# VGLoic/kzg-poly-commit-exploration

Hardware: AMD Instinct MI355X
Metric: g1_msm_commitments_per_sec_degree_2^20 (higher is better)
Workload: dtype i32 digits (Fp: 13 signed radix-2^30 digits, Montgomery 2^390; Fr: 8 x u32, Montgomery 2^256)

## Files before the change

### kzg_poly_commit_exploration_amd/csrc/api.hip

```cpp
#include <hip/hip_runtime.h>
#include <sys/random.h>

#include <algorithm>
#include <atomic>
#include <cerrno>
#include <chrono>
#include <condition_variable>
#include <cstdio>
#include <cstdlib>
#include <cstring>
#include <deque>
#include <functional>
#include <mutex>
#include <new>
#include <string>
#include <thread>
#include <vector>

#include "../../include/kzg_mi355x.h"
#include "engine.h"
#include "host_field.hpp"
#include "host_fr.hpp"
#include "fr30_host.hpp"
#include "host_pairing.hpp"
#include "host_sha256.hpp"
#include "wire30.hip.h"

using namespace kzg;
namespace hf = kzg_host;

namespace {

constexpr size_t kMaxCoefficients = 0xFFFFFFFFull;

#ifndef KZG_NUM_SLOTS
#define KZG_NUM_SLOTS 5
#endif
constexpr int kNumSlots = KZG_NUM_SLOTS;
struct ReducePlan {
    uint32_t lo_bits = 0, hi_bits = 0;
    uint32_t row_lo = 0, row_hi = 0;
    uint32_t col_lo = 0, col_hi = 0;
    uint32_t off_r2row = 0, off_c2row = 0, off_r2col = 0, off_c2col = 0, total = 0;
};

enum SlotKind { SLOT_IDLE = 0, SLOT_COMMIT = 1, SLOT_OPEN = 2, SLOT_TRIVIAL = 3, SLOT_COMMIT_BATCH = 4, SLOT_OPEN_BATCH = 5, SLOT_RESERVED = 6,
                SLOT_OPEN_POINTS = 7 ,
                SLOT_OPEN_COMBINED = 8 ,
                SLOT_OPEN_SETS = 9  };

int hip_fail(kzg_ctx* ctx, const char* what, hipError_t e);

struct DevBuf {
    void* p = nullptr;
    size_t cap = 0;
    DevBuf() = default;
    DevBuf(const DevBuf&) = delete;
    DevBuf& operator=(const DevBuf&) = delete;
    ~DevBuf() { reset(); }
    void reset() {
        if (p) hipFree(p);
        p = nullptr;
        cap = 0;
    }
    template <class T = uint32_t> T* dev() const { return (T*)p; }
    int reserve(kzg_ctx* ctx, size_t bytes, hipStream_t drain = nullptr) { return bytes <= cap ? KZG_OK : grow(ctx, bytes, drain); }
    int grow(kzg_ctx* ctx, size_t bytes, hipStream_t drain) {
        if (drain)
            if (hipError_t e = hipStreamSynchronize(drain)) return hip_fail(ctx, "hipStreamSynchronize", e);
        reset();
        if (hipError_t e = hipMalloc(&p, bytes)) {
            p = nullptr;
            return hip_fail(ctx, "hipMalloc", e);
        }
// ... 74 lines not shown
    DevBuf recoded;
    DevBuf part_a, part_b;
    DevBuf pair_scratch;
    DevBuf heavy_ws;
    DevBuf arena;
    PinnedBuf fin{PinnedBuf::Mapped};
    DevBuf stage;
    DevBuf q;
    DevBuf chunk, block;
    PinnedBuf small{PinnedBuf::Mapped};
    PinnedBuf bsmall{PinnedBuf::Mapped};
    std::vector<uint32_t> open_ys;
    PinnedBuf roots{PinnedBuf::Staged};
    PinnedBuf pvals{PinnedBuf::Mapped};
    DevBuf pblock;
    std::vector<uint32_t> pts_ys;
    size_t pts_nq = 0;
    PinnedBuf ctab{PinnedBuf::Staged};
    PinnedBuf cvals{PinnedBuf::Mapped};
    DevBuf cpart, cin;
    size_t cmb_t = 0;
    float combine_ms = 0;
    PinnedBuf stab{PinnedBuf::Staged}, ssel{PinnedBuf::Staged};
    PinnedBuf svals{PinnedBuf::Mapped};
    DevBuf sg;
    std::vector<uint32_t> sets_vmap;
    PinnedBuf ltab{PinnedBuf::Staged};
    PinnedBuf btab{PinnedBuf::Staged};
    DevBuf lag_part;
    DevBuf gp_in, gp_z, gp_part;
    PinnedBuf gp_flags{PinnedBuf::Mapped};
    DevBuf cpoly, cagg;
    DevBuf ml_in, ml_pyr;
    SlotKind kind = SLOT_IDLE;
    size_t job_n = 0;
    uint32_t job_batch = 1;
    uint32_t open_y[8] = {};
    bool timing = false;
    bool has_quotient = false;
    bool tail_checked = false;
    kzg_kernel_times times = {};
};

}

struct kzg_ctx {
    kzg::MultiState* multi = nullptr;
    int device = 0;
    std::mutex mu;
    std::condition_variable slot_cv;
    int sync_owned = 0;
    bool raw_partials = false;
    bool host_trace = false;
    std::atomic<uint64_t> trace_ns[5] = {};
    std::atomic<uint64_t> trace_calls{0};
    std::string last_error;
    size_t n = 0;
    MsmConfig cfg = {};
    DevBuf table;
    bool nttb_ready = false;
    DevBuf ntt_tw;
    DevBuf lag_table;
    size_t lag_n = 0;
    uint64_t srs_gen = 0;
    ReducePlan plan;
    size_t arena_records = 0, final_records = 0;
    uint32_t max_batch = 1;
    Slot slots[kNumSlots];
    hipStream_t front_stream = nullptr, heavy_stream = nullptr, tail_stream = nullptr;
    hipStream_t upload_stream = nullptr;
    uint32_t accum_lds_bytes = 41u * 1024u;
    uint32_t small_lds_bytes = 48u * 1024u;
    bool small_msm_off = false;
    size_t pq_ws_budget = (size_t)1 << 30;
    bool slots_ready = false;
    bool timing = false;
    std::mutex fk20_mu;
    DevBuf glv;
    uint32_t glv_log = 0;
    DevBuf fk20_B, fk20_tab;
    uint32_t fk20_log_L = 0, fk20_log_l = 0;
    Workspace<11> fk20_ws;
    std::mutex recover_mu;
    DevBuf rec_g;
    Workspace<11> rec_ws;
    Workspace<17> vc_ws;
    Workspace<8> blob_ws;
    std::mutex lookup_mu;
    Workspace<6> lu_ws;
    std::mutex quotient_mu;
    Workspace<13> pq_ws;
    DevBuf prove_buf[5];
    uint32_t pq_zinv_key = ~0u;
    std::vector<kzg_circuit*> circuits;
};

struct kzg_circuit {
    kzg_ctx* owner = nullptr;
    uint32_t lg_n = 0, lg_ext = 0;
    size_t n = 0, t = 0;
    size_t c_tab = 0;
    size_t g_custom = 0, d_max = 0;
    uint8_t exps[kCgMaxTerms * kPqMaxColumns] = {};
    uint8_t exps_next[kCgMaxTerms * kPqMaxColumns] = {};
    size_t rho = 0;
    uint8_t next_wires[kPqMaxColumns] = {};
    uint64_t shifts[4 * kPqMaxColumns] = {};
    DevBuf values;
// ... 188 lines not shown

int build_tables(kzg_ctx* ctx, hipStream_t st, void* d_xyzz_tmp, void* d_prefix) {
    const size_t n = ctx->n;
    for (uint32_t j = 1; j < ctx->cfg.W; j++) {
        char* prev = (char*)ctx->table.p + (size_t)(j - 1) * n * kAffineBytes;
        char* next = (char*)ctx->table.p + (size_t)j * n * kAffineBytes;
        launch_table_window(st, prev, (uint32_t)n, ctx->cfg.level_bits, d_xyzz_tmp, d_prefix, next);
    }
    HIP_TRY(ctx, hipGetLastError());
    HIP_TRY(ctx, hipStreamSynchronize(st));
    return KZG_OK;
}

int drain_all(kzg_ctx* ctx) {
    for (hipStream_t st : {ctx->upload_stream, ctx->front_stream, ctx->heavy_stream, ctx->tail_stream})
        if (st) HIP_TRY(ctx, hipStreamSynchronize(st));
    return KZG_OK;
}

static int srs_release(kzg_ctx* ctx) {
    ctx->slots_ready = false;
    int rc = drain_all(ctx);
    if (rc) return rc;
    for (auto& s : ctx->slots) s.kind = SLOT_IDLE;
    ctx->table.reset();
    ctx->fk20_B.reset();
    ctx->fk20_tab.reset();
    ctx->lag_table.reset();
    ctx->lag_n = 0;
    ctx->srs_gen++;
    ctx->n = 0;
    return KZG_OK;
}

int srs_prepare(kzg_ctx* ctx, size_t n) {
    if (n == 0 || n > 0x7fffffffu / 32) return KZG_ERR_INVALID_ARG;
    int rc = srs_release(ctx);
    if (rc) return rc;
    size_t free_b = 0, total_b = 0;
    HIP_TRY(ctx, hipMemGetInfo(&free_b, &total_b));
    size_t budget = (size_t)((double)free_b * 0.6);
    if (const char* v = std::getenv("KZG_TABLE_GB")) budget = (size_t)(std::strtod(v, nullptr) * 1073741824.0);
    MsmConfig cfg = choose_msm_config(n, budget);
    if ((size_t)cfg.W * n >= 0x80000000ull) return KZG_ERR_INVALID_ARG;
    ctx->cfg = cfg;
    return ctx->table.reserve(ctx, (size_t)cfg.W * n * kAffineBytes);
}

struct MsmBasis {
    const void* table;
    uint32_t stride;
};
int enqueue_msm(kzg_ctx* ctx, Slot& s, const uint32_t* d_scalars, int is_mont, size_t n, int ev_base,
                uint32_t batch = 1, uint64_t stride = 0, const MsmBasis* basis = nullptr) {
    const MsmConfig cfg = ctx->cfg;
    const void* table = basis ? basis->table : ctx->table.p;
    const uint32_t table_stride = basis ? basis->stride : (uint32_t)ctx->n;
    const uint32_t nbt = cfg.nb * batch;
    hipStream_t st = s.stream;
    s.end = st;
    if (s.timing) HIP_TRY(ctx, hipEventRecord(s.ev[ev_base], st));
    const bool header_zeroed = launch_bucket_sort(st, d_scalars, is_mont, (uint32_t)n, batch, stride, table_stride, cfg, s.cnt.dev(),
                       s.block_sums.dev(), s.pairs.dev<uint64_t>(), s.recoded.dev(), s.offs.dev(), s.sorted.dev(), (uint32_t*)s.heavy_ws.p);
    if (s.timing) {
        HIP_TRY(ctx, hipEventRecord(s.ev[ev_base + 1], st));
        HIP_TRY(ctx, hipEventRecord(s.ev[ev_base + 2], st));
    }
    bool alone = true;
    for (const auto& other : ctx->slots) alone = alone && (&other == &s || other.kind == SLOT_IDLE);
    const uint64_t max_refs = (uint64_t)n * cfg.max_digits * batch;
    const uint32_t lanes = accumulate_lanes(max_refs, alone);
    const ReducePlan& P = ctx->plan;
    const uint32_t R = 1u << P.hi_bits, C = 1u << P.lo_bits, B = batch;
    char* row = (char*)s.arena.p;
    char* col = row + (size_t)R * B * kXyzzBytes;
    char* fin = (char*)s.fin.d;
    const uint32_t rl = 1u << P.row_lo, rh = 1u << P.row_hi, cl = 1u << P.col_lo, ch = 1u << P.col_hi;
    const TreeSumDesc stage1[2] = {
        {s.buckets.p, row, B * R, C, C, 1, B * R, 0},
        {s.buckets.p, col, B * C, R, 1, C, C, (uint64_t)cfg.nb}};
    const TreeSumDesc stage2[4] = {
        {row, fin + (size_t)P.off_r2row * B * kXyzzBytes, B * rh, rl, rl, 1, rh, R},
        {row, fin + (size_t)P.off_c2row * B * kXyzzBytes, B * rl, rh, 1, rl, rl, R},
        {col, fin + (size_t)P.off_r2col * B * kXyzzBytes, B * ch, cl, cl, 1, ch, C},
        {col, fin + (size_t)P.off_c2col * B * kXyzzBytes, B * cl, ch, 1, cl, cl, C}};
    if (!header_zeroed) HIP_TRY(ctx, hipMemsetAsync(s.heavy_ws.p, 0, kHeavyHeaderBytes, st));
    if (max_refs <= kTinyRefs && !ctx->small_msm_off) {
        if (s.timing) HIP_TRY(ctx, hipEventRecord(s.ev[ev_base + 3], st));
        launch_small_msm(st, table, s.sorted.dev(), s.offs.dev(), nbt, lanes, max_refs, s.buckets.p, s.part_a.p, s.part_b.p,
                         s.heavy_ws.p, s.small.dev() + 26, stage1, stage2, ctx->small_lds_bytes);
        if (s.timing) HIP_TRY(ctx, hipEventRecord(s.ev[ev_base + 4], st));
    } else {
        const bool hand_over = !alone;
        hipStream_t hs = hand_over ? ctx->heavy_stream : st;
        if (hand_over) {
            HIP_TRY(ctx, hipEventRecord(s.sorted_ev, st));
            HIP_TRY(ctx, hipStreamWaitEvent(hs, s.sorted_ev, 0));
        }
        if (s.timing) HIP_TRY(ctx, hipEventRecord(s.ev[ev_base + 3], hs));
        launch_bucket_accumulate(hs, table, s.sorted.dev(), s.offs.dev(), nbt, lanes, s.buckets.p, s.part_a.p, s.part_b.p,
                                 ctx->accum_lds_bytes, s.pair_scratch.p, max_refs,
                                 (char*)s.heavy_ws.p + kAccumClockOffset);
        if (s.timing) HIP_TRY(ctx, hipEventRecord(s.ev[ev_base + 4], hs));
        if (hand_over) {
            HIP_TRY(ctx, hipEventRecord(s.accum_ev, hs));
            st = s.end = ctx->tail_stream;
            HIP_TRY(ctx, hipStreamWaitEvent(st, s.accum_ev, 0));
        }
        launch_bucket_finalize(st, s.offs.dev(), nbt, lanes, s.part_a.p, s.part_b.p, s.buckets.p, s.heavy_ws.p, s.small.dev() + 26,
                               finalize_group_size(nbt));
        launch_tree_sums_two_stage(st, stage1, 2, stage2, 4, (uint32_t*)s.heavy_ws.p + 64, alone);
    }
    if (s.timing) HIP_TRY(ctx, hipEventRecord(s.ev[ev_base + 5], st));
    HIP_TRY(ctx, hipGetLastError());
    return KZG_OK;
}

hf::PX host_wsum(const uint64_t* recs, uint32_t len) {
    hf::PX run = hf::px_inf(), acc = hf::px_inf();
    for (uint32_t v = len; v-- > 1;) {
        run = hf::px_add(run, hf::px_from_record(recs + (size_t)v * kXyzzWords64));
        acc = hf::px_add(acc, run);
    }
    return acc;
}
hf::PX host_shift(hf::PX p, uint32_t k) {
    for (uint32_t i = 0; i < k; i++) p = hf::px_double(p);
    return p;
}
hf::P1 finish_msm(const kzg_ctx* ctx, const Slot& s, uint32_t p = 0, uint32_t batch = 1) {
    const ReducePlan& P = ctx->plan;
    const uint64_t* f = s.fin.host<uint64_t>();
    auto at = [&](uint32_t off, uint32_t len) { return f + ((size_t)off * batch + (size_t)p * len) * kXyzzWords64; };
    const uint32_t rh = 1u << P.row_hi, rl = 1u << P.row_lo, ch = 1u << P.col_hi, cl = 1u << P.col_lo;
    hf::PX w_row = hf::px_add(host_shift(host_wsum(at(P.off_r2row, rh), rh), P.row_lo), host_wsum(at(P.off_c2row, rl), rl));
    hf::PX w_col = hf::px_add(host_shift(host_wsum(at(P.off_r2col, ch), ch), P.col_lo), host_wsum(at(P.off_c2col, cl), cl));
    hf::PX total = hf::px_add(host_shift(w_row, P.lo_bits), w_col);
    if (ctx->cfg.recode == kRecodeNaf) total = hf::px_double(total);
    const uint64_t* r2 = at(P.off_r2row, rh);
    for (uint32_t k = 0; k < rh; k++) total = hf::px_add(total, hf::px_from_record(r2 + (size_t)k * kXyzzWords64));
    return ctx->raw_partials ? hf::px_to_jacobian(total) : hf::px_normalize(total);
}

void write_p1(uint64_t out[18], const hf::P1& p) { std::memcpy(out, &p, sizeof p); }

void fill_device_times(Slot& s) {
    s.times.references = s.small.host()[26];
    const uint64_t not_start = (uint64_t)s.small.host()[28] | ((uint64_t)s.small.host()[29] << 32);
    const uint64_t end = (uint64_t)s.small.host()[30] | ((uint64_t)s.small.host()[31] << 32);
    if (not_start != 0 && end > ~not_start) s.times.accumulate_ms = (float)((double)(end - ~not_start) * 1e-5);
}
void fill_accumulate_times(Slot& s) {
    float ms = 0;
    (void)hipEventElapsedTime(&ms, s.ev[3], s.ev[4]);
    s.times.accumulate_events_ms = ms;
    if (s.times.accumulate_ms == 0) s.times.accumulate_ms = ms;
}

void slot_idle(kzg_ctx* ctx, Slot& s) {
    s.kind = SLOT_IDLE;
    ctx->slot_cv.notify_all();
}
int reserve_slot(kzg_ctx* ctx, std::unique_lock<std::mutex>& lk, bool block) {
    for (;;) {
        for (int i = 0; i < kNumSlots; i++)
            if (ctx->slots[i].kind == SLOT_IDLE) {
                ctx->slots[i].kind = SLOT_RESERVED;
                ctx->sync_owned++;
                return i;
            }
        if (!block || ctx->sync_owned == 0) return -1;
        ctx->slot_cv.wait(lk);
    }
}
void release_owned(kzg_ctx* ctx, int slot) {
    if (ctx->slots[slot].kind == SLOT_RESERVED) ctx->slots[slot].kind = SLOT_IDLE;
    ctx->sync_owned--;
    ctx->slot_cv.notify_all();
}
struct SlotLease {
    kzg_ctx* ctx;
    int slot;
    ~SlotLease() { if (slot >= 0) release_owned(ctx, slot); }
};
void quiesce(kzg_ctx* ctx, std::unique_lock<std::mutex>& lk) {
    while (ctx->sync_owned > 0) ctx->slot_cv.wait(lk);
}

bool host_tail_nonzero(const uint64_t* coeffs, size_t from, size_t n) {
    for (size_t i = from; i < n; i++)
        if (coeffs[4 * i] | coeffs[4 * i + 1] | coeffs[4 * i + 2] | coeffs[4 * i + 3]) return true;
    return false;
}
// ... 70 lines not shown
        case KZG_ERR_CONSTANT_POLY: return "Unable to divide a constant polynomial";
        case KZG_ERR_REMAINDER:
            return "[divide_by_root] Fail to divide the polynomial by a root, constant terms do not add up";
        case KZG_ERR_INVALID_ARG: return "invalid argument";
        case KZG_ERR_NO_DEVICE: return "no HIP device available (this library has no CPU path)";
        case KZG_ERR_HIP: return "HIP runtime error";
        case KZG_ERR_NO_SRS: return "no SRS loaded";
        case KZG_ERR_BUSY: return "slot busy";
        default: return "unknown status";
    }
}

const char* kzg_last_error(const kzg_ctx* ctx) {
    if (!ctx) return "";
    if (ctx->multi && ctx->last_error.empty()) return multi_last_error(ctx->multi);
    return ctx->last_error.c_str();
}

int kzg_ctx_create_multi_ex(const int* devices, int ndev, unsigned flags, kzg_ctx** out) {
    if (!out) return KZG_ERR_INVALID_ARG;
    *out = nullptr;
    if (!devices || ndev <= 0 || (flags & ~(unsigned)KZG_MULTI_REPLICATE_SRS)) return KZG_ERR_INVALID_ARG;
    kzg::MultiState* m = nullptr;
    std::string err;
    int rc = multi_create(devices, ndev, (flags & KZG_MULTI_REPLICATE_SRS) ? kMultiReplicate : kMultiRange, &m, err);
    if (rc != KZG_OK) return rc;
    kzg_ctx* ctx = new kzg_ctx();
    ctx->multi = m;
    ctx->device = devices[0];
    *out = ctx;
    return KZG_OK;
}
int kzg_ctx_create_multi(const int* devices, int ndev, kzg_ctx** out) { return kzg_ctx_create_multi_ex(devices, ndev, 0u, out); }
int kzg_abi_version(void) { return KZG_ABI_VERSION; }
int kzg_num_devices(const kzg_ctx* ctx) { return !ctx ? 0 : (ctx->multi ? multi_num_devices(ctx->multi) : 1); }
uint64_t kzg_rccl_exchanges(const kzg_ctx* ctx) { return (ctx && ctx->multi) ? multi_rccl_exchanges(ctx->multi) : 0; }

int kzg_ctx_create(int device, kzg_ctx** out) {
    if (!out) return KZG_ERR_INVALID_ARG;
    *out = nullptr;
    int count = 0;
    if (hipGetDeviceCount(&count) != hipSuccess || count <= 0) return KZG_ERR_NO_DEVICE;
    if (device < 0 || device >= count) return KZG_ERR_NO_DEVICE;
    if (hipSetDevice(device) != hipSuccess) return KZG_ERR_NO_DEVICE;
    kzg_ctx* ctx = new kzg_ctx();
    ctx->device = device;
    if (const char* v = std::getenv("KZG_ACCUM_LDS_KB")) ctx->accum_lds_bytes = (uint32_t)std::atoi(v) * 1024u;
    if (const char* v = std::getenv("KZG_SMALL_MSM")) ctx->small_msm_off = std::atoi(v) == 0;
    if (const char* v = std::getenv("KZG_PQ_WS_KB")) {
        const long kb = std::atol(v);
        ctx->pq_ws_budget = kb < 0 ? 0 : (kb > (1l << 20) ? (size_t)1 << 30 : (size_t)kb * 1024);
    }
    if (const char* v = std::getenv("KZG_HOST_TRACE")) ctx->host_trace = std::atoi(v) != 0;
    if (hipFuncSetAttribute(small_msm_kernel(), hipFuncAttributeMaxDynamicSharedMemorySize, (int)small_msm_lds_bytes()) == hipSuccess)
        ctx->small_lds_bytes = small_msm_lds_bytes();
    else
        (void)hipGetLastError();
    if (!poly_prepare_device() || !points_prepare_device() || !sets_prepare_device()) {
        delete ctx;
        return KZG_ERR_HIP;
    }
    *out = ctx;
    return KZG_OK;
}

void kzg_ctx_destroy(kzg_ctx* ctx) {
    if (!ctx) return;
    if (ctx->multi) {
        multi_destroy(ctx->multi);
        delete ctx;
        return;
    }
    hipSetDevice(ctx->device);
    if (ctx->host_trace && ctx->trace_calls.load()) {
        const double k = 1e-3 / (double)ctx->trace_calls.load();
        std::fprintf(stderr, "[kzg host trace] %llu kzg_commit calls, us per call: wait-for-slot %.1f upload %.1f submit %.1f device %.1f collect %.1f\n",
                     (unsigned long long)ctx->trace_calls.load(), k * ctx->trace_ns[0].load(), k * ctx->trace_ns[1].load(),
                     k * ctx->trace_ns[2].load(), k * ctx->trace_ns[3].load(), k * ctx->trace_ns[4].load());
    }
    for (hipStream_t st : {ctx->upload_stream, ctx->front_stream, ctx->heavy_stream, ctx->tail_stream})
        if (st) hipStreamSynchronize(st);
    for (hipStream_t st : {ctx->upload_stream, ctx->front_stream, ctx->heavy_stream, ctx->tail_stream})
        if (st) hipStreamDestroy(st);
    for (kzg_circuit* c : ctx->circuits) delete c;
    delete ctx;
}

size_t kzg_srs_len(const kzg_ctx* ctx) { return !ctx ? 0 : (ctx->multi ? multi_srs_len(ctx->multi) : ctx->n); }
int kzg_num_slots(const kzg_ctx*) { return kNumSlots; }

int kzg_msm_config(const kzg_ctx* ctx, int* digit_bits, int* table_levels, size_t* num_buckets, int* recoding) {
    if (ctx && ctx->multi)
        return kzg_msm_config(multi_kid(ctx->multi, 0), digit_bits, table_levels, num_buckets, recoding);
    if (!ctx || !ctx->n) return KZG_ERR_NO_SRS;
    if (digit_bits) *digit_bits = (int)ctx->cfg.c;
    if (table_levels) *table_levels = (int)ctx->cfg.W;
    if (num_buckets) *num_buckets = ctx->cfg.nb;
    if (recoding) *recoding = (int)ctx->cfg.recode;
    return KZG_OK;
}

int kzg_srs_load_g1(kzg_ctx* ctx, const void* first_g1, size_t stride, size_t n) {
    if (!ctx || !first_g1 || stride < 144) return KZG_ERR_INVALID_ARG;
    if (ctx->multi) {
        std::lock_guard<std::mutex> lkm(ctx->mu);
        ctx->last_error.clear();
        return n ? multi_srs_load(ctx->multi, first_g1, stride, n) : KZG_ERR_INVALID_ARG;
    }
    std::unique_lock<std::mutex> lk(ctx->mu);
    quiesce(ctx, lk);
    HIP_TRY(ctx, hipSetDevice(ctx->device));
    int rc = srs_prepare(ctx, n);
    if (rc) return rc;
    std::vector<uint64_t> packed(n * 18);
    for (size_t i = 0; i < n; i++) std::memcpy(&packed[i * 18], (const char*)first_g1 + i * stride, 144);
    DevBuf d_jac, d_prefix, d_xyzz;
    HIP_TRY(ctx, hipMalloc(&d_jac.p, n * 144));
    HIP_TRY(ctx, hipMalloc(&d_prefix.p, n * 64));
    HIP_TRY(ctx, hipMalloc(&d_xyzz.p, n * kXyzzBytes));
    TmpStream st;
    HIP_TRY(ctx, hipStreamCreateWithFlags(&st.s, hipStreamNonBlocking));
    HIP_TRY(ctx, hipMemcpyAsync(d_jac.p, packed.data(), n * 144, hipMemcpyHostToDevice, st.s));
    ctx->n = n;
    launch_jacobian_to_affine(st.s, d_jac.p, (uint32_t)n, ctx->table.p, d_prefix.p);
    rc = build_tables(ctx, st.s, d_xyzz.p, d_prefix.p);
    if (rc) {
        ctx->n = 0;
        return rc;
    }
    return setup_slots(ctx);
}
// ... 196 lines not shown
    if (ok) {
        ok = std::fseek(f, 0, SEEK_END) == 0;
        const long end = ok ? std::ftell(f) : -1;
        ok = ok && end >= 0 && (uint64_t)end == 128ull + 96ull * h.n && std::fseek(f, 128, SEEK_SET) == 0;
    }
    std::vector<uint64_t> xy;
    if (ok) {
        try {
            xy.resize((size_t)h.n * 12);
        } catch (const std::bad_alloc&) {
            std::fclose(f);
            return fail("out of host memory for the SRS file");
        }
        ok = std::fread(xy.data(), 96, h.n, f) == h.n;
    }
    std::fclose(f);
    if (ok) {
        uint8_t a[48], b[48];
        affine96_compress(xy.data(), a);
        affine96_compress(&xy[12 * ((size_t)h.n - 1)], b);
        ok = std::memcmp(a, h.first, 48) == 0 && std::memcmp(b, h.last, 48) == 0;
    }
    if (!ok) return fail("not a KZGSRS1 file, truncated, or its fingerprint does not match its content");
    size_t bad = 0;
    if (!affine96_all_on_curve(xy.data(), (size_t)h.n, &bad)) return fail("SRS file: point " + std::to_string(bad) + " is not on the curve");
    return kzg_srs_load_affine(ctx, xy.data(), (size_t)h.n);
}

int kzg_srs_read_g1(kzg_ctx* ctx, size_t index, size_t count, uint64_t* out_p1) {
    if (!ctx || !out_p1) return KZG_ERR_INVALID_ARG;
    std::lock_guard<std::mutex> lk(ctx->mu);
    if (ctx->multi) return multi_srs_len(ctx->multi) ? multi_srs_read(ctx->multi, index, count, out_p1) : KZG_ERR_NO_SRS;
    if (!ctx->n) return KZG_ERR_NO_SRS;
    if (index > ctx->n || count > ctx->n - index) return KZG_ERR_INVALID_ARG;
    if (!count) return KZG_OK;
    HIP_TRY(ctx, hipSetDevice(ctx->device));
    DevBuf d_p1;
    HIP_TRY(ctx, hipMalloc(&d_p1.p, count * 144));
    hipStream_t st = ctx->slots[0].stream;
    launch_affine_to_p1(st, (const char*)ctx->table.p + index * kAffineBytes, (uint32_t)count, d_p1.p);
    HIP_TRY(ctx, hipMemcpyAsync(out_p1, d_p1.p, count * 144, hipMemcpyDeviceToHost, st));
    HIP_TRY(ctx, hipStreamSynchronize(st));
    return KZG_OK;
}


static bool lagrange_basis(const kzg_ctx* ctx, size_t n, MsmBasis* out) {
    if (!ctx->lag_table.p || ctx->lag_n != n) return false;
    *out = MsmBasis{ctx->lag_table.p, (uint32_t)ctx->lag_n};
    return true;
}

static int submit_commit_locked(kzg_ctx* ctx, int slot, const uint32_t* d_scalars, int is_mont, size_t n,
                                bool tail_already_checked, bool owned = false, const MsmBasis* basis = nullptr) {
    if (!ctx->n || !ctx->slots_ready) return KZG_ERR_NO_SRS;
    if (basis && (basis->stride != n || n > ctx->n)) return KZG_ERR_INVALID_ARG;
    if (slot < 0 || slot >= kNumSlots) return KZG_ERR_INVALID_ARG;
    Slot& s = ctx->slots[slot];
    if (s.kind != (owned ? SLOT_RESERVED : SLOT_IDLE)) return KZG_ERR_BUSY;
    HIP_TRY(ctx, hipSetDevice(ctx->device));
    s.timing = ctx->timing;
    s.end = s.stream;
    s.has_quotient = false;
    s.job_n = n;
    s.job_batch = 1;
    s.tail_checked = tail_already_checked;
    std::memset(&s.times, 0, sizeof s.times);
    size_t n_msm = n < ctx->n ? n : ctx->n;
    std::memset(s.small.host(), 0, 64 * 4);
    if (n > ctx->n && !tail_already_checked) {
        uint64_t cnt = n - ctx->n;
        hipLaunchKernelGGL(k_tail_nonzero, dim3((unsigned)((cnt + 255) / 256)), dim3(256), 0, s.stream, d_scalars,
                           (uint64_t)ctx->n, (uint64_t)n, s.small.dev() + 24);
    }
    if (n_msm == 0) {
        s.kind = SLOT_TRIVIAL;
        return KZG_OK;
    }
    int rc = enqueue_msm(ctx, s, d_scalars, is_mont, n_msm, 0, 1, 0, basis);
    if (rc) return rc;
    HIP_TRY(ctx, hipEventRecord(s.done, s.end));
    s.kind = SLOT_COMMIT;
    return KZG_OK;
}

int kzg_commit_submit(kzg_ctx* ctx, int slot, const void* d_coeffs, size_t n) {
    KZG_SINGLE_DEVICE_ONLY(ctx);
    if (!ctx || (!d_coeffs && n)) return KZG_ERR_INVALID_ARG;
    if (n > kMaxCoefficients) return KZG_ERR_INVALID_ARG;
    std::lock_guard<std::mutex> lk(ctx->mu);
    return submit_commit_locked(ctx, slot, (const uint32_t*)d_coeffs, 1, n, false);
}

static int submit_open_locked(kzg_ctx* ctx, int slot, const uint32_t* d_coeffs, size_t n, const uint64_t z[4],
                              const uint64_t y[4], bool owned = false) {
    if (!ctx->n || !ctx->slots_ready) return KZG_ERR_NO_SRS;
    if (slot < 0 || slot >= kNumSlots) return KZG_ERR_INVALID_ARG;
    Slot& s = ctx->slots[slot];
    if (s.kind != (owned ? SLOT_RESERVED : SLOT_IDLE)) return KZG_ERR_BUSY;
    HIP_TRY(ctx, hipSetDevice(ctx->device));
    int rc = ensure_poly(ctx, s, n);
    if (rc) return rc;
    s.timing = ctx->timing;
    s.end = s.stream;
    s.job_n = n;
    s.job_batch = 1;
    s.has_quotient = true;
    s.tail_checked = false;
    std::memcpy(s.open_y, y, 32);
    std::memset(&s.times, 0, sizeof s.times);
    if (n == 0) {
        std::memset(s.small.host(), 0, 64 * 4);
        s.kind = SLOT_TRIVIAL;
        return KZG_OK;
    }
    uint32_t zw[8];
    std::memcpy(zw, z, 32);
    if (s.timing) HIP_TRY(ctx, hipEventRecord(s.ev[6], s.stream));
    if (!launch_quotient_single(s.stream, d_coeffs, (uint32_t)n, zw, n > 1 ? s.q.dev() : nullptr, s.small.dev())) {
        std::memset(s.small.host(), 0, 64 * 4);
        PolyScratch sc{s.chunk.dev(), s.block.dev(), s.small.dev(), s.small.dev() + 8};
        launch_quotient(s.stream, d_coeffs, (uint32_t)n, zw, n > 1 ? s.q.dev() : nullptr, sc);
    }
    if (s.timing) HIP_TRY(ctx, hipEventRecord(s.ev[7], s.stream));
    size_t nq = n - 1;
    if (nq > ctx->n) {
        uint64_t from = ctx->n + 1, cnt = n - from;
        hipLaunchKernelGGL(k_tail_nonzero, dim3((unsigned)((cnt + 255) / 256)), dim3(256), 0, s.stream, d_coeffs, from,
                           (uint64_t)n, s.small.dev() + 24);
        nq = ctx->n;
    }
    if (nq > 0) {
// ... 13 lines not shown
    return submit_open_locked(ctx, slot, (const uint32_t*)d_coeffs, n, z, y);
}

static int submit_points_locked(kzg_ctx* ctx, int slot, const uint32_t* d_coeffs, size_t n, const uint64_t* zs,
                                const uint64_t* ys, size_t k, bool owned = false) {
    if (!ctx->n || !ctx->slots_ready) return KZG_ERR_NO_SRS;
    if (slot < 0 || slot >= kNumSlots) return KZG_ERR_INVALID_ARG;
    Slot& s = ctx->slots[slot];
    if (s.kind != (owned ? SLOT_RESERVED : SLOT_IDLE)) return KZG_ERR_BUSY;
    uint64_t ws[4 * KZG_MAX_OPEN_POINTS];
    int rc = points_weights(ctx, zs, k, ws);
    if (rc) return rc;
    HIP_TRY(ctx, hipSetDevice(ctx->device));
    rc = ensure_poly(ctx, s, n);
    if (rc == KZG_OK) rc = ensure_points(ctx, s, n, k);
    if (rc) return rc;
    s.timing = ctx->timing;
    s.end = s.stream;
    s.job_n = n;
    s.job_batch = 1;
    s.has_quotient = true;
    s.tail_checked = false;
    s.pts_ys.assign((const uint32_t*)ys, (const uint32_t*)ys + 8 * k);
    std::memset(&s.times, 0, sizeof s.times);
    size_t nq = n > k ? n - k : 0;
    if (s.timing) HIP_TRY(ctx, hipEventRecord(s.ev[6], s.stream));
    rc = enqueue_points_scan(ctx, s, d_coeffs, n, zs, ws, k, nq, nq > 0);
    if (rc) return rc;
    if (s.timing) HIP_TRY(ctx, hipEventRecord(s.ev[7], s.stream));
    if (nq > ctx->n) {
        const uint64_t from = ctx->n + k, cnt = n - from;
        hipLaunchKernelGGL(k_tail_nonzero, dim3((unsigned)((cnt + 255) / 256)), dim3(256), 0, s.stream, d_coeffs, from,
                           (uint64_t)n, s.small.dev() + 24);
        nq = ctx->n;
    }
    if (nq > 0) {
        rc = enqueue_msm(ctx, s, s.q.dev(), 1, nq, 0);
        if (rc) return rc;
    }
    s.pts_nq = nq;
    HIP_TRY(ctx, hipEventRecord(s.done, s.end));
    s.kind = SLOT_OPEN_POINTS;
    return KZG_OK;
}

int kzg_open_points_submit(kzg_ctx* ctx, int slot, const void* d_coeffs, size_t n, const uint64_t* zs, const uint64_t* ys,
                           size_t k) {
    KZG_SINGLE_DEVICE_ONLY(ctx);
    if (!ctx || !zs || !ys || (!d_coeffs && n) || n > kMaxCoefficients) return KZG_ERR_INVALID_ARG;
    std::lock_guard<std::mutex> lk(ctx->mu);
    return submit_points_locked(ctx, slot, (const uint32_t*)d_coeffs, n, zs, ys, k);
}

static int wait_locked(kzg_ctx* ctx, int slot, uint64_t out_p1[18]) {
    if (slot < 0 || slot >= kNumSlots) return KZG_ERR_INVALID_ARG;
    Slot& s = ctx->slots[slot];
    if (s.kind == SLOT_IDLE) return KZG_ERR_INVALID_ARG;
    if (s.kind == SLOT_COMMIT_BATCH || s.kind == SLOT_OPEN_BATCH) {
        ctx->last_error = "kzg_wait on a slot that holds a batched job (use kzg_wait_batch / kzg_wait_open_batch)";
        return KZG_ERR_INVALID_ARG;
    }
    if (s.kind == SLOT_OPEN_COMBINED) {
        ctx->last_error = "kzg_wait on a slot that holds a combined opening (use kzg_wait_combined)";
        return KZG_ERR_INVALID_ARG;
    }
    if (s.kind == SLOT_OPEN_SETS) {
        ctx->last_error = "kzg_wait on a slot that holds an opening at several point sets (use kzg_wait_sets)";
        return KZG_ERR_INVALID_ARG;
    }
    if (s.kind == SLOT_RESERVED) return KZG_ERR_BUSY;
    HIP_TRY(ctx, hipSetDevice(ctx->device));
    SlotKind kind = s.kind;
    slot_idle(ctx, s);
    HIP_TRY(ctx, hipEventSynchronize(s.done));
    const bool ran_msm = kind != SLOT_TRIVIAL && !(kind == SLOT_OPEN_POINTS && s.pts_nq == 0);
    if (ran_msm) fill_device_times(s);
    if (s.timing && ran_msm) {
        float ms = 0;
        hipEventElapsedTime(&ms, s.ev[0], s.ev[1]); s.times.digits_ms = ms;
        hipEventElapsedTime(&ms, s.ev[2], s.ev[3]); s.times.scatter_ms = ms;
        fill_accumulate_times(s);
        hipEventElapsedTime(&ms, s.ev[4], s.ev[5]); s.times.reduce_ms = ms;
        if (s.has_quotient) {
            hipEventElapsedTime(&ms, s.ev[6], s.ev[7]); s.times.quotient_ms = ms;
            hipEventElapsedTime(&ms, s.ev[6], s.ev[5]); s.times.total_ms = ms;
        } else {
            hipEventElapsedTime(&ms, s.ev[0], s.ev[5]); s.times.total_ms = ms;
        }
    }
    const uint32_t* hs = s.small.host();
    hf::P1 inf = hf::p1_inf();
    if (kind == SLOT_OPEN_POINTS) {
        const size_t k = s.pts_ys.size() / 8;
        const uint32_t* vals = points_values(s, k);
        for (size_t i = 0; i < k; i++)
            if (std::memcmp(vals + 8 * i, s.pts_ys.data() + 8 * i, 32) != 0) return KZG_ERR_REMAINDER;
        if (hs[24]) return KZG_ERR_DEGREE_TOO_HIGH;
        write_p1(out_p1, s.pts_nq ? finish_msm(ctx, s) : inf);
        return KZG_OK;
    }
    if (s.has_quotient) {
        const size_t n = s.job_n;
        if (n == 0) {
            bool y_zero = true;
            for (int i = 0; i < 8; i++) y_zero &= s.open_y[i] == 0;
            if (!y_zero) return KZG_ERR_CONSTANT_POLY;
            write_p1(out_p1, inf);
            return KZG_OK;
        }
        bool higher_nonzero = hs[0] & 1u;
        if (!higher_nonzero) {
            if (std::memcmp(hs + 16, s.open_y, 32) != 0) return KZG_ERR_CONSTANT_POLY;
            write_p1(out_p1, inf);
            return KZG_OK;
        }
        if (std::memcmp(hs + 8, s.open_y, 32) != 0) return KZG_ERR_REMAINDER;
        if (hs[24]) return KZG_ERR_DEGREE_TOO_HIGH;
    } else {
        if (hs[24]) return KZG_ERR_DEGREE_TOO_HIGH;
    }
    if (kind == SLOT_TRIVIAL) {
        write_p1(out_p1, inf);
        return KZG_OK;
    }
    write_p1(out_p1, finish_msm(ctx, s));
    return KZG_OK;
}

int kzg_set_max_batch(kzg_ctx* ctx, size_t max_batch) {
    if (!ctx || max_batch == 0) return KZG_ERR_INVALID_ARG;
    if (ctx->multi) return multi_set_max_batch(ctx->multi, max_batch);
    std::unique_lock<std::mutex> lk(ctx->mu);
    quiesce(ctx, lk);
    HIP_TRY(ctx, hipSetDevice(ctx->device));
    int rc = drain_all(ctx);
    if (rc) return rc;
    for (auto& s : ctx->slots)
        if (s.kind != SLOT_IDLE) return KZG_ERR_BUSY;
    const uint32_t previous = ctx->max_batch;
    ctx->max_batch = (uint32_t)(max_batch > 1024 ? 1024 : max_batch);
    if (!ctx->n) return KZG_OK;
    rc = setup_slots(ctx, true);
    if (rc != KZG_OK) {
        const std::string why = ctx->last_error;
        ctx->max_batch = previous;
        (void)hipGetLastError();
        (void)setup_slots(ctx);
        ctx->last_error = why;
    }
    return rc;
}

size_t kzg_max_batch(const kzg_ctx* ctx) {
    if (ctx && ctx->multi) return kzg_max_batch(multi_kid(ctx->multi, 0));
    return ctx ? ctx->max_batch : 0;
}

static int commit_batch_submit_locked(kzg_ctx* ctx, int slot, const void* d_coeffs, size_t n, size_t batch,
                                      size_t stride_coeffs, bool owned = false, bool lagrange = false) {
    if (!ctx->n || !ctx->slots_ready) return KZG_ERR_NO_SRS;
    MsmBasis basis{};
    if (lagrange && !lagrange_basis(ctx, n, &basis)) return KZG_ERR_NO_SRS;
    if (slot < 0 || slot >= kNumSlots || batch > ctx->max_batch) return KZG_ERR_INVALID_ARG;
    if (n > ctx->n) return KZG_ERR_DEGREE_TOO_HIGH;
    Slot& s = ctx->slots[slot];
    if (s.kind != (owned ? SLOT_RESERVED : SLOT_IDLE)) return KZG_ERR_BUSY;
    HIP_TRY(ctx, hipSetDevice(ctx->device));
    s.timing = ctx->timing;
    s.end = s.stream;
    s.has_quotient = false;
    s.job_n = n;
    s.job_batch = (uint32_t)batch;
    s.tail_checked = true;
// ... 122 lines not shown
    const hf::P1 inf = hf::p1_inf();
    for (uint32_t p = 0; p < B; p++) {
        const uint32_t* hs = s.bsmall.host() + p * 32;
        const uint32_t* y = s.open_ys.data() + 8 * p;
        uint64_t* out = out_p1s + out_stride * (size_t)p;
        int& status = statuses[status_stride * (size_t)p];
        if (!(hs[0] & 1u)) {
            if (std::memcmp(hs + 16, y, 32) != 0) status = KZG_ERR_CONSTANT_POLY;
            else { status = KZG_OK; write_p1(out, inf); }
            continue;
        }
        if (std::memcmp(hs + 8, y, 32) != 0) { status = KZG_ERR_REMAINDER; continue; }
        status = KZG_OK;
        write_p1(out, finish_msm(ctx, s, p, B));
    }
    s.open_ys.clear();
    return KZG_OK;
}

int kzg_wait_open_batch(kzg_ctx* ctx, int slot, uint64_t* out_p1s, int* statuses, size_t batch) {
    KZG_SINGLE_DEVICE_ONLY(ctx);
    if (!ctx || !out_p1s || !statuses) return KZG_ERR_INVALID_ARG;
    std::lock_guard<std::mutex> lk(ctx->mu);
    return wait_open_batch_locked(ctx, slot, out_p1s, statuses, batch);
}

int kzg_wait(kzg_ctx* ctx, int slot, uint64_t out_p1[18]) {
    KZG_SINGLE_DEVICE_ONLY(ctx);
    if (!ctx || !out_p1) return KZG_ERR_INVALID_ARG;
    std::lock_guard<std::mutex> lk(ctx->mu);
    return wait_locked(ctx, slot, out_p1);
}


static void await_unlocked(std::unique_lock<std::mutex>& lk, Slot& s) {
    if (s.kind == SLOT_TRIVIAL || s.kind == SLOT_RESERVED || s.kind == SLOT_IDLE) return;
    lk.unlock();
    (void)hipEventSynchronize(s.done);
    lk.lock();
}

struct HostTrace {
    kzg_ctx* ctx;
    std::chrono::steady_clock::time_point t;
    explicit HostTrace(kzg_ctx* c) : ctx(c) { if (c->host_trace) t = std::chrono::steady_clock::now(); }
    void mark(int phase) {
        if (!ctx->host_trace) return;
        const auto now = std::chrono::steady_clock::now();
        ctx->trace_ns[phase] += (uint64_t)std::chrono::duration_cast<std::chrono::nanoseconds>(now - t).count();
        t = now;
    }
};

static int commit_host(kzg_ctx* ctx, const void* scalars, int is_mont, size_t n, uint64_t out_p1[18]) {
    if (!ctx || !out_p1 || (!scalars && n)) return KZG_ERR_INVALID_ARG;
    if (n > kMaxCoefficients) return KZG_ERR_INVALID_ARG;
    if (ctx->multi) return multi_commit(ctx->multi, scalars, is_mont, n, out_p1);
    HostTrace tr(ctx);
    std::unique_lock<std::mutex> lk(ctx->mu);
    if (!ctx->n || !ctx->slots_ready) return KZG_ERR_NO_SRS;
    HIP_TRY(ctx, hipSetDevice(ctx->device));
    if (n > ctx->n && host_tail_nonzero((const uint64_t*)scalars, ctx->n, n)) return KZG_ERR_DEGREE_TOO_HIGH;
    const int slot = reserve_slot(ctx, lk, true);
    if (slot < 0) return KZG_ERR_BUSY;
    Slot& s = ctx->slots[slot];
    const size_t n_dev = n < ctx->n ? n : ctx->n;
    int rc = ensure_poly(ctx, s, n_dev);
    tr.mark(0);
    if (rc == KZG_OK) rc = upload_unlocked(ctx, lk, s, s.stage.dev(), scalars, n_dev * 32);
    tr.mark(1);
    if (rc == KZG_OK) rc = submit_commit_locked(ctx, slot, s.stage.dev(), is_mont, n_dev, true, true);
    tr.mark(2);
    if (rc == KZG_OK) {
        await_unlocked(lk, s);
        tr.mark(3);
        rc = wait_locked(ctx, slot, out_p1);
        tr.mark(4);
    }
    release_owned(ctx, slot);
    ctx->trace_calls++;
    return rc;
}

int kzg_commit(kzg_ctx* ctx, const uint64_t* coeffs, size_t n, uint64_t out_p1[18]) {
    return commit_host(ctx, coeffs, 1, n, out_p1);
}
int kzg_commit_le_bytes(kzg_ctx* ctx, const uint8_t* scalars_le, size_t n, uint64_t out_p1[18]) {
    return commit_host(ctx, scalars_le, 0, n, out_p1);
}

int kzg_open(kzg_ctx* ctx, const uint64_t* coeffs, size_t n, const uint64_t z[4], const uint64_t y[4],
             uint64_t out_p1[18]) {
    if (!ctx || !out_p1 || !z || !y || (!coeffs && n)) return KZG_ERR_INVALID_ARG;
    if (n > kMaxCoefficients) return KZG_ERR_INVALID_ARG;
    if (ctx->multi) return multi_open(ctx->multi, coeffs, n, z, y, out_p1);
    std::unique_lock<std::mutex> lk(ctx->mu);
    if (!ctx->n || !ctx->slots_ready) return KZG_ERR_NO_SRS;
    HIP_TRY(ctx, hipSetDevice(ctx->device));
    const int slot = reserve_slot(ctx, lk, true);
    if (slot < 0) return KZG_ERR_BUSY;
    Slot& s = ctx->slots[slot];
    int rc = ensure_poly(ctx, s, n);
    if (rc == KZG_OK) rc = upload_unlocked(ctx, lk, s, s.stage.dev(), coeffs, n * 32);
    if (rc == KZG_OK) rc = submit_open_locked(ctx, slot, s.stage.dev(), n, z, y, true);
    if (rc == KZG_OK) {
        await_unlocked(lk, s);
        rc = wait_locked(ctx, slot, out_p1);
    }
    release_owned(ctx, slot);
    return rc;
}

int kzg_open_points(kzg_ctx* ctx, const uint64_t* coeffs, size_t n, const uint64_t* zs, const uint64_t* ys, size_t k,
                    uint64_t out_p1[18]) {
    if (!ctx || !out_p1 || !zs || !ys || (!coeffs && n) || n > kMaxCoefficients) return KZG_ERR_INVALID_ARG;
    if (k < 1 || k > KZG_MAX_OPEN_POINTS) return KZG_ERR_INVALID_ARG;
    if (ctx->multi) return multi_open_points(ctx->multi, coeffs, n, zs, ys, k, out_p1);
    std::unique_lock<std::mutex> lk(ctx->mu);
    if (!ctx->n || !ctx->slots_ready) return KZG_ERR_NO_SRS;
    HIP_TRY(ctx, hipSetDevice(ctx->device));
    const int slot = reserve_slot(ctx, lk, true);
    if (slot < 0) return KZG_ERR_BUSY;
    Slot& s = ctx->slots[slot];
    int rc = ensure_poly(ctx, s, n);
    if (rc == KZG_OK) rc = upload_unlocked(ctx, lk, s, s.stage.dev(), coeffs, n * 32);
    if (rc == KZG_OK) rc = submit_points_locked(ctx, slot, s.stage.dev(), n, zs, ys, k, true);
    if (rc == KZG_OK) {
        await_unlocked(lk, s);
        rc = wait_locked(ctx, slot, out_p1);
    }
    release_owned(ctx, slot);
    return rc;
// ... 8586 lines not shown
```

Measured before the change: 435.0.

## Split large single commits into ranges to overlap upload with MSM

For single commits at or above a threshold (default 2^19), the scalar range is split across two idle slots, 25% first and 75% second. The first range's MSM runs on its own basis view while the second range uploads, and the partial results are summed on the host. This aims to hide the host-to-device transfer behind kernel work. In exchange it adds extra kernel launches and bucket reductions, and the ranges compete for the GPU because neither slot counts as alone.

```diff
diff --git a/kzg_poly_commit_exploration_amd/csrc/api.hip b/kzg_poly_commit_exploration_amd/csrc/api.hip
--- a/kzg_poly_commit_exploration_amd/csrc/api.hip
+++ b/kzg_poly_commit_exploration_amd/csrc/api.hip
@@ -20,6 +20,7 @@
 #include "../../include/kzg_mi355x.h"
 #include "engine.h"
 #include "host_field.hpp"
+#include "host_split.hpp"
 #include "host_fr.hpp"
 #include "fr30_host.hpp"
 #include "host_pairing.hpp"
@@ -200,8 +201,9 @@
     int sync_owned = 0;
     bool raw_partials = false;
     bool host_trace = false;
-    std::atomic<uint64_t> trace_ns[5] = {};
-    std::atomic<uint64_t> trace_calls{0};
+    std::atomic<uint64_t> trace_ns[6] = {};
+    std::atomic<uint64_t> trace_calls{0}, trace_split_calls{0};
+    kzg_split::Knobs host_split;
     std::string last_error;
     size_t n = 0;
     MsmConfig cfg = {};
@@ -496,7 +498,7 @@
     uint32_t stride;
 };
 int enqueue_msm(kzg_ctx* ctx, Slot& s, const uint32_t* d_scalars, int is_mont, size_t n, int ev_base,
-                uint32_t batch = 1, uint64_t stride = 0, const MsmBasis* basis = nullptr) {
+                uint32_t batch = 1, uint64_t stride = 0, const MsmBasis* basis = nullptr, bool lone_tail = false) {
     const MsmConfig cfg = ctx->cfg;
     const void* table = basis ? basis->table : ctx->table.p;
     const uint32_t table_stride = basis ? basis->stride : (uint32_t)ctx->n;
@@ -553,7 +555,7 @@
         }
         launch_bucket_finalize(st, s.offs.dev(), nbt, lanes, s.part_a.p, s.part_b.p, s.buckets.p, s.heavy_ws.p, s.small.dev() + 26,
                                finalize_group_size(nbt));
-        launch_tree_sums_two_stage(st, stage1, 2, stage2, 4, (uint32_t*)s.heavy_ws.p + 64, alone);
+        launch_tree_sums_two_stage(st, stage1, 2, stage2, 4, (uint32_t*)s.heavy_ws.p + 64, alone || lone_tail);
     }
     if (s.timing) HIP_TRY(ctx, hipEventRecord(s.ev[ev_base + 5], st));
     HIP_TRY(ctx, hipGetLastError());
@@ -572,7 +574,7 @@
     for (uint32_t i = 0; i < k; i++) p = hf::px_double(p);
     return p;
 }
-hf::P1 finish_msm(const kzg_ctx* ctx, const Slot& s, uint32_t p = 0, uint32_t batch = 1) {
+hf::PX finish_msm_px(const kzg_ctx* ctx, const Slot& s, uint32_t p = 0, uint32_t batch = 1) {
     const ReducePlan& P = ctx->plan;
     const uint64_t* f = s.fin.host<uint64_t>();
     auto at = [&](uint32_t off, uint32_t len) { return f + ((size_t)off * batch + (size_t)p * len) * kXyzzWords64; };
@@ -583,6 +585,10 @@
     if (ctx->cfg.recode == kRecodeNaf) total = hf::px_double(total);
     const uint64_t* r2 = at(P.off_r2row, rh);
     for (uint32_t k = 0; k < rh; k++) total = hf::px_add(total, hf::px_from_record(r2 + (size_t)k * kXyzzWords64));
+    return total;
+}
+hf::P1 finish_msm(const kzg_ctx* ctx, const Slot& s, uint32_t p = 0, uint32_t batch = 1) {
+    const hf::PX total = finish_msm_px(ctx, s, p, batch);
     return ctx->raw_partials ? hf::px_to_jacobian(total) : hf::px_normalize(total);
 }
 
@@ -759,6 +765,7 @@
         ctx->pq_ws_budget = kb < 0 ? 0 : (kb > (1l << 20) ? (size_t)1 << 30 : (size_t)kb * 1024);
     }
     if (const char* v = std::getenv("KZG_HOST_TRACE")) ctx->host_trace = std::atoi(v) != 0;
+    ctx->host_split = kzg_split::parse_knobs(std::getenv("KZG_HOST_SPLIT"));
     if (hipFuncSetAttribute(small_msm_kernel(), hipFuncAttributeMaxDynamicSharedMemorySize, (int)small_msm_lds_bytes()) == hipSuccess)
         ctx->small_lds_bytes = small_msm_lds_bytes();
     else
@@ -781,9 +788,11 @@
     hipSetDevice(ctx->device);
     if (ctx->host_trace && ctx->trace_calls.load()) {
         const double k = 1e-3 / (double)ctx->trace_calls.load();
-        std::fprintf(stderr, "[kzg host trace] %llu kzg_commit calls, us per call: wait-for-slot %.1f upload %.1f submit %.1f device %.1f collect %.1f\n",
+        std::fprintf(stderr, "[kzg host trace] %llu kzg_commit calls, us per call: wait-for-slot %.1f upload %.1f submit %.1f device %.1f collect %.1f"
+                     " | %llu range-split, upload hidden under kernels %.1f\n",
                      (unsigned long long)ctx->trace_calls.load(), k * ctx->trace_ns[0].load(), k * ctx->trace_ns[1].load(),
-                     k * ctx->trace_ns[2].load(), k * ctx->trace_ns[3].load(), k * ctx->trace_ns[4].load());
+                     k * ctx->trace_ns[2].load(), k * ctx->trace_ns[3].load(), k * ctx->trace_ns[4].load(),
+                     (unsigned long long)ctx->trace_split_calls.load(), k * ctx->trace_ns[5].load());
     }
     for (hipStream_t st : {ctx->upload_stream, ctx->front_stream, ctx->heavy_stream, ctx->tail_stream})
         if (st) hipStreamSynchronize(st);
@@ -1086,9 +1095,10 @@
 }
 
 static int submit_commit_locked(kzg_ctx* ctx, int slot, const uint32_t* d_scalars, int is_mont, size_t n,
-                                bool tail_already_checked, bool owned = false, const MsmBasis* basis = nullptr) {
+                                bool tail_already_checked, bool owned = false, const MsmBasis* basis = nullptr,
+                                bool lone_tail = false) {
     if (!ctx->n || !ctx->slots_ready) return KZG_ERR_NO_SRS;
-    if (basis && (basis->stride != n || n > ctx->n)) return KZG_ERR_INVALID_ARG;
+    if (basis && (basis->stride < n || n > ctx->n)) return KZG_ERR_INVALID_ARG;
     if (slot < 0 || slot >= kNumSlots) return KZG_ERR_INVALID_ARG;
     Slot& s = ctx->slots[slot];
     if (s.kind != (owned ? SLOT_RESERVED : SLOT_IDLE)) return KZG_ERR_BUSY;
@@ -1111,7 +1121,7 @@
         s.kind = SLOT_TRIVIAL;
         return KZG_OK;
     }
-    int rc = enqueue_msm(ctx, s, d_scalars, is_mont, n_msm, 0, 1, 0, basis);
+    int rc = enqueue_msm(ctx, s, d_scalars, is_mont, n_msm, 0, 1, 0, basis, lone_tail);
     if (rc) return rc;
     HIP_TRY(ctx, hipEventRecord(s.done, s.end));
     s.kind = SLOT_COMMIT;
@@ -1231,7 +1241,7 @@
     return submit_points_locked(ctx, slot, (const uint32_t*)d_coeffs, n, zs, ys, k);
 }
 
-static int wait_locked(kzg_ctx* ctx, int slot, uint64_t out_p1[18]) {
+static int wait_locked(kzg_ctx* ctx, int slot, uint64_t out_p1[18], bool no_point = false) {
     if (slot < 0 || slot >= kNumSlots) return KZG_ERR_INVALID_ARG;
     Slot& s = ctx->slots[slot];
     if (s.kind == SLOT_IDLE) return KZG_ERR_INVALID_ARG;
@@ -1298,6 +1308,7 @@
     } else {
         if (hs[24]) return KZG_ERR_DEGREE_TOO_HIGH;
     }
+    if (no_point) return KZG_OK;
     if (kind == SLOT_TRIVIAL) {
         write_p1(out_p1, inf);
         return KZG_OK;
@@ -1526,6 +1537,42 @@
     }
 };
 
+static int commit_host_ranges(kzg_ctx* ctx, std::unique_lock<std::mutex>& lk, HostTrace& tr, const int* slots, int k,
+                              const void* scalars, int is_mont, size_t n_dev, uint64_t out_p1[18]) {
+    const kzg_split::Plan plan = kzg_split::plan_ranges(n_dev, k, ctx->host_split.first_permille);
+    k = plan.k;
+    int rc = KZG_OK;
+    for (int r = 0; r < k && rc == KZG_OK; r++) rc = ensure_poly(ctx, ctx->slots[slots[r]], plan.len[r]);
+    tr.mark(0);
+    int submitted = 0;
+    for (int r = 0; r < k && rc == KZG_OK; r++) {
+        Slot& s = ctx->slots[slots[r]];
+        rc = upload_unlocked(ctx, lk, s, s.stage.dev(), (const char*)scalars + plan.lo[r] * 32, plan.len[r] * 32);
+        tr.mark(r == 0 ? 1 : 5);
+        if (rc) break;
+        const MsmBasis view{(const char*)ctx->table.p + plan.lo[r] * kAffineBytes, (uint32_t)ctx->n};
+        rc = submit_commit_locked(ctx, slots[r], s.stage.dev(), is_mont, plan.len[r], true, true, &view, r == k - 1);
+        tr.mark(2);
+        if (rc == KZG_OK) submitted++;
+    }
+    hf::PX parts[kzg_split::kMaxRanges];
+    for (int r = 0; r < submitted; r++) {
+        const Slot& s = ctx->slots[slots[r]];
+        await_unlocked(lk, ctx->slots[slots[r]]);
+        tr.mark(3);
+        parts[r] = s.kind == SLOT_COMMIT ? finish_msm_px(ctx, s) : hf::px_inf();
+        tr.mark(4);
+    }
+    for (int r = 0; r < submitted; r++) {
+        const int rc_r = wait_locked(ctx, slots[r], nullptr, true);
+        if (rc == KZG_OK) rc = rc_r;
+    }
+    if (rc == KZG_OK) write_p1(out_p1, kzg_split::combine_partials(parts, k));
+    tr.mark(4);
+    ctx->trace_split_calls++;
+    return rc;
+}
+
 static int commit_host(kzg_ctx* ctx, const void* scalars, int is_mont, size_t n, uint64_t out_p1[18]) {
     if (!ctx || !out_p1 || (!scalars && n)) return KZG_ERR_INVALID_ARG;
     if (n > kMaxCoefficients) return KZG_ERR_INVALID_ARG;
@@ -1539,19 +1586,36 @@
     if (slot < 0) return KZG_ERR_BUSY;
     Slot& s = ctx->slots[slot];
     const size_t n_dev = n < ctx->n ? n : ctx->n;
-    int rc = ensure_poly(ctx, s, n_dev);
-    tr.mark(0);
-    if (rc == KZG_OK) rc = upload_unlocked(ctx, lk, s, s.stage.dev(), scalars, n_dev * 32);
-    tr.mark(1);
-    if (rc == KZG_OK) rc = submit_commit_locked(ctx, slot, s.stage.dev(), is_mont, n_dev, true, true);
-    tr.mark(2);
-    if (rc == KZG_OK) {
-        await_unlocked(lk, s);
-        tr.mark(3);
-        rc = wait_locked(ctx, slot, out_p1);
-        tr.mark(4);
-    }
-    release_owned(ctx, slot);
+    int rc = KZG_OK;
+    int slots[kzg_split::kMaxRanges] = {slot, -1, -1, -1};
+    int k = 1;
+    if (ctx->host_split.on() && n_dev >= ctx->host_split.threshold && !ctx->raw_partials) {
+        bool others_idle = true;
+        for (int i = 0; i < kNumSlots; i++) others_idle = others_idle && (i == slot || ctx->slots[i].kind == SLOT_IDLE);
+        const int want = kzg_split::plan_ranges(n_dev, ctx->host_split.k, ctx->host_split.first_permille).k;
+        while (others_idle && k < want) {
+            const int more = reserve_slot(ctx, lk, false);
+            if (more < 0) break;
+            slots[k++] = more;
+        }
+    }
+    if (k > 1) {
+        rc = commit_host_ranges(ctx, lk, tr, slots, k, scalars, is_mont, n_dev, out_p1);
+    } else {
+        rc = ensure_poly(ctx, s, n_dev);
+        tr.mark(0);
+        if (rc == KZG_OK) rc = upload_unlocked(ctx, lk, s, s.stage.dev(), scalars, n_dev * 32);
+        tr.mark(1);
+        if (rc == KZG_OK) rc = submit_commit_locked(ctx, slot, s.stage.dev(), is_mont, n_dev, true, true);
+        tr.mark(2);
+        if (rc == KZG_OK) {
+            await_unlocked(lk, s);
+            tr.mark(3);
+            rc = wait_locked(ctx, slot, out_p1);
+            tr.mark(4);
+        }
+    }
+    for (int r = 0; r < k; r++) release_owned(ctx, slots[r]);
     ctx->trace_calls++;
     return rc;
 }
diff --git a/kzg_poly_commit_exploration_amd/csrc/host_split.hpp b/kzg_poly_commit_exploration_amd/csrc/host_split.hpp
--- /dev/null
+++ b/kzg_poly_commit_exploration_amd/csrc/host_split.hpp
@@ -0,0 +1,74 @@
+#pragma once
+#include <cstddef>
+#include <cstdlib>
+
+#include "host_field.hpp"
+
+namespace kzg_split {
+
+constexpr int kMaxRanges = 4;
+constexpr unsigned kMinFirstPermille = 1, kMaxFirstPermille = 999;
+
+struct Plan {
+    int k = 0;
+    size_t lo[kMaxRanges] = {}, len[kMaxRanges] = {};
+};
+
+inline Plan plan_ranges(size_t n, int k, unsigned first_permille) {
+    Plan p;
+    if (n == 0) return p;
+    if (k < 1) k = 1;
+    if (k > kMaxRanges) k = kMaxRanges;
+    if ((size_t)k > n) k = (int)n;
+    p.k = k;
+    if (k == 1) {
+        p.len[0] = n;
+        return p;
+    }
+    if (first_permille < kMinFirstPermille) first_permille = kMinFirstPermille;
+    if (first_permille > kMaxFirstPermille) first_permille = kMaxFirstPermille;
+    size_t first = (size_t)((unsigned __int128)n * first_permille / 1000u);
+    const size_t later = (size_t)k - 1;
+    if (first < 1) first = 1;
+    if (first > n - later) first = n - later;
+    p.len[0] = first;
+    const size_t rest = n - first, each = rest / later, longer = rest % later;
+    for (size_t r = 1; r <= later; r++) {
+        p.lo[r] = p.lo[r - 1] + p.len[r - 1];
+        p.len[r] = each + (r <= longer ? 1 : 0);
+    }
+    return p;
+}
+
+struct Knobs {
+    size_t threshold = (size_t)1 << 19;
+    int k = 2;
+    unsigned first_permille = 250;
+    bool on() const { return threshold != 0 && k > 1; }
+};
+inline Knobs parse_knobs(const char* v, Knobs d = Knobs()) {
+    if (!v || !*v) return d;
+    char* end = nullptr;
+    const unsigned long long t = std::strtoull(v, &end, 10);
+    if (end == v) return d;
+    d.threshold = (size_t)t;
+    if (*end != ':') return d;
+    const char* f = end + 1;
+    const long k = std::strtol(f, &end, 10);
+    if (end == f) return d;
+    d.k = k < 1 ? 1 : (k > kMaxRanges ? kMaxRanges : (int)k);
+    if (*end != ':') return d;
+    f = end + 1;
+    const long s = std::strtol(f, &end, 10);
+    if (end == f) return d;
+    d.first_permille = s < (long)kMinFirstPermille ? kMinFirstPermille : (s > (long)kMaxFirstPermille ? kMaxFirstPermille : (unsigned)s);
+    return d;
+}
+
+inline kzg_host::P1 combine_partials(const kzg_host::PX* parts, int k) {
+    kzg_host::PX total = kzg_host::px_inf();
+    for (int r = 0; r < k; r++) total = kzg_host::px_add(total, parts[r]);
+    return kzg_host::px_normalize(total);
+}
+
+}
```

Result: no change. 439.5 (median of 4 runs) (+1.0%).
